# yuecideng/Misc3D

Hardware: AMD Instinct MI355X
Metric: RANSAC hypotheses/sec, 1M-pt cloud (inlier-score GB/s: roofline.algorithmic_reuse) (higher is better)
Workload: dtype f64 decisions (fp32 screen + fp64 recount)

## Files before the change

### include/misc3d_amd.h

```cpp
#ifndef MISC3D_AMD_H
#define MISC3D_AMD_H

#include <stddef.h>
#include <stdint.h>

#ifdef __cplusplus
extern "C" {
#endif

#define M3D_OK 1
#define M3D_FALSE 0
#define M3D_ERR_PROBABILITY (-1)
#define M3D_ERR_TOO_FEW_POINTS (-2)
#define M3D_ERR_NO_NORMALS (-3)
#define M3D_ERR_SIZE_MISMATCH (-4)
#define M3D_ERR_INVALID_ARG (-5)
#define M3D_ERR_DEVICE (-6)
#define M3D_ERR_INTERNAL (-7)

enum m3d_model_kind { M3D_PLANE = 0, M3D_SPHERE = 1, M3D_CYLINDER = 2 };

typedef struct m3d_stats {
    double fitness;
    double inlier_rmse;
// ... 326 lines not shown
    int32_t lead_hypotheses;
    int32_t score_groups_per_block;
    int32_t score_min_workgroups;
    int32_t dense_workgroups;
    int32_t reg_neighbour_lists;
    int32_t reg_prune;
    int32_t match_brute;
    int32_t match_fp32_screen;
    int32_t pool_limit_mb;
    int32_t kernel_timing;
    int32_t reg_sorted_lists;
    int32_t score_fp32_screen;
    int32_t cull_fp32;
    int32_t reg_fp32_screen;
    int32_t sorted_tombstones;
    int32_t score_mfma;
    int32_t score_mfma_groups;
    int32_t score_waves4;
    int32_t score_waves4_groups;
    int32_t score_phases;
    int32_t compact_one_pass;
    int32_t plane_bound;
    int32_t lanes;
    int32_t wait_spin_us;
    int32_t prestream;
    int32_t chunk_cap;
    int32_t first_chunk;
    int32_t reg_cells_per_radius;
    int32_t match_pipeline;
    int32_t reg_cache;
    int32_t device_aliases;
    int32_t lanes_eager;
    int32_t list_mask;
} m3d_config;
void m3d_get_config(m3d_config *out);
int m3d_set_config(const m3d_config *in);

const char *m3d_last_error(void);
int m3d_device_count(void);
const char *m3d_version(void);

#ifdef __cplusplus
}
#endif
#endif
```

### misc3d_amd/capi.py

```python
from __future__ import annotations

import ctypes as C
import threading
import os
import sys
from dataclasses import dataclass

import numpy as np

_HERE = os.path.dirname(os.path.abspath(__file__))
FP_ORDER = int(os.environ.get("M3D_FP_ORDER", "0") or 0)
_VARIANT = os.environ.get("M3D_LIB_VARIANT", "")
LIB_PATH = os.path.join(_HERE, "lib", *([_VARIANT] if _VARIANT else ([f"order{FP_ORDER}"] if FP_ORDER else [])), "libmisc3d_amd.so")
HEADER_PATH = os.path.join(os.path.dirname(_HERE), "include", "misc3d_amd.h")

PLANE, SPHERE, CYLINDER = 0, 1, 2
MINIMAL_SAMPLE = {PLANE: 3, SPHERE: 4, CYLINDER: 2}
NUM_PARAMS = {PLANE: 4, SPHERE: 4, CYLINDER: 7}
MODEL_STRIDE = 8

OK, FALSE = 1, 0
ERR_PROBABILITY, ERR_TOO_FEW_POINTS, ERR_NO_NORMALS, ERR_SIZE_MISMATCH = -1, -2, -3, -4
ERR_INVALID_ARG, ERR_DEVICE, ERR_INTERNAL = -5, -6, -7

# ... 173 lines not shown
                                                          C.c_void_p, C.c_int, C.c_size_t, C.c_void_p, C.c_void_p,
                                                          C.c_void_p, C.c_void_p, C.c_void_p]
        L.m3d_segment_plane_iterative_sharded.argtypes = [C.c_void_p, C.c_size_t, C.c_double, C.c_int, C.c_double,
                                                          C.c_void_p, C.c_int, C.c_void_p, C.c_size_t, C.c_void_p,
                                                          C.c_void_p, C.c_void_p, C.c_void_p]
        L.m3d_segment_plane_iterative_multi.argtypes = [C.c_void_p, C.c_size_t, C.c_double, C.c_int, C.c_double,
                                                        C.c_void_p, C.c_void_p, C.c_int, C.c_size_t, C.c_void_p,
                                                        C.c_void_p, C.c_void_p, C.c_void_p]
        L.m3d_fit_multi.argtypes = [C.c_int, C.c_void_p, C.c_void_p, C.c_size_t, C.c_double, C.c_size_t, C.c_double,
                                    C.c_void_p, C.c_void_p, C.c_int, C.c_void_p, C.c_void_p, C.c_void_p, C.c_void_p]
        L.m3d_registration_ransac_sharded.argtypes = [C.c_void_p, C.c_size_t, C.c_void_p, C.c_size_t, C.c_void_p,
                                                      C.c_void_p, C.c_size_t, C.c_double, C.c_int, C.c_double,
                                                      C.c_double, C.c_void_p, C.c_int, C.c_void_p, C.c_void_p,
                                                      C.c_void_p]
        L.m3d_bench_fp64_issue_rate.argtypes = [C.c_int, C.c_double, C.c_void_p, C.c_void_p]
        L.m3d_bench_cloud_setup_ms.argtypes = [C.c_void_p, C.c_void_p]
        L.m3d_bench_last_segment_ms.argtypes = [C.c_void_p]
        L.m3d_bench_reg_checkers.argtypes = [C.c_void_p, C.c_void_p, C.c_void_p, C.c_double, C.c_double]
        L.m3d_get_config.restype = None
        L.m3d_get_config.argtypes = [C.c_void_p]
        L.m3d_set_config.argtypes = [C.c_void_p]
        L.m3d_release_cached.restype = None
        L.m3d_release_cached.argtypes = [C.c_int]
        _lib = L
    return _lib


class Config(C.Structure):
    _fields_ = [(k, C.c_int32) for k in ("dense_scoring", "speculative_refine", "lead_hypotheses",
                                         "score_groups_per_block", "score_min_workgroups", "dense_workgroups",
                                         "reg_neighbour_lists", "reg_prune", "match_brute", "match_fp32_screen",
                                         "pool_limit_mb", "kernel_timing", "reg_sorted_lists", "score_fp32_screen",
                                         "cull_fp32", "reg_fp32_screen", "sorted_tombstones", "score_mfma", "score_mfma_groups", "score_waves4", "score_waves4_groups", "score_phases", "compact_one_pass", "plane_bound",
                                         "lanes", "wait_spin_us", "prestream", "chunk_cap", "first_chunk", "reg_cells_per_radius", "match_pipeline", "reg_cache", "device_aliases", "lanes_eager", "list_mask")]


def fp64_issue_rate(device=0, ms_target=2.0):
    t, ms = C.c_double(0), C.c_double(0)
    _check(lib().m3d_bench_fp64_issue_rate(device, ms_target, C.cast(C.byref(t), C.c_void_p), C.cast(C.byref(ms), C.c_void_p)))
    return float(t.value), float(ms.value)


def mfma_probe(xyz512, box, max_abs, records, device=0):
    xyz = np.ascontiguousarray(xyz512, dtype=np.float64).reshape(512, 3)
    bx = np.ascontiguousarray(box, dtype=np.float64).reshape(6)
    rec = np.zeros((len(records), 8), dtype=np.float64)
    rec[:, :5] = np.asarray(records, dtype=np.float64).reshape(-1, 5)
    q = np.empty((len(rec), 512, 2), dtype=np.float64)
    h = np.empty((len(rec), 3), dtype=np.float64)
    off = np.empty((512, 3), dtype=np.float32)
    f = lib().m3d_bench_mfma_probe
    f.restype = C.c_int
    f.argtypes = [C.c_int, C.c_void_p, C.c_void_p, C.c_double, C.c_void_p, C.c_size_t, C.c_void_p, C.c_void_p, C.c_void_p]
    _check(f(device, xyz.ctypes.data, bx.ctypes.data, float(max_abs), rec.ctypes.data, len(rec), q.ctypes.data, h.ctypes.data,
             off.ctypes.data))
    return q, h[:, 0].copy(), h[:, 1].copy(), h[:, 2].copy(), off


def match_last_path() -> int:
    f = lib().m3d_bench_match_last_path
    f.restype = C.c_uint
    f.argtypes = []
    return int(f())


def experimental() -> bool:
    f = lib().m3d_bench_experimental
# ... 1130 lines not shown
```

### misc3d_amd/csrc/m3d_config.cpp

```cpp
#include "m3d_config.hpp"

#include <algorithm>
#include <cstdlib>
#include <cstring>
#include <mutex>

#include "m3d_driver.hpp"

namespace m3d {
namespace {
m3d_config g_cfg;
std::once_flag g_once;
std::mutex g_cfg_mu;
thread_local m3d_config t_cfg;
thread_local int t_cfg_pins = 0;

long env_long(const char* name, long def) {
    const char* e = std::getenv(name);
    if (!e || !*e) return def;
    char* end = nullptr;
    const long v = std::strtol(e, &end, 10);
    return end == e ? def : v;
}
bool env_is(const char* name, char first) {
    const char* e = std::getenv(name);
    return e && e[0] == first;
}
void sanitize(m3d_config& c) {
    if (c.lead_hypotheses < 64 || c.lead_hypotheses % 64) c.lead_hypotheses = 128;
    if (c.score_groups_per_block < 1 || c.score_groups_per_block > 64) c.score_groups_per_block = 8;
    if (c.score_min_workgroups < 1) c.score_min_workgroups = 8192;
    if (c.dense_workgroups < 1) c.dense_workgroups = 8192;
    if (c.pool_limit_mb < 0) c.pool_limit_mb = 0;
    if (c.score_mfma_groups < 1 || c.score_mfma_groups > 64) c.score_mfma_groups = 64;
    if (c.score_waves4_groups < 1 || c.score_waves4_groups > 64) c.score_waves4_groups = 64;
    if (c.score_phases < -1 || c.score_phases == 1 || c.score_phases > 3) c.score_phases = -1;
    if (c.plane_bound < 0 || c.plane_bound > 2) c.plane_bound = 1;
    if (c.cull_fp32 < 0 || c.cull_fp32 > 2) c.cull_fp32 = 1;
    if (!kExperimentalBuild) c.score_mfma = c.score_waves4 = c.compact_one_pass = 0;
    if (c.lanes < 1 || c.lanes > 8) c.lanes = 4;
    if (c.wait_spin_us < 0) c.wait_spin_us = 500;
    c.prestream = c.prestream != 0;
    c.chunk_cap = (int32_t)std::min<long>(std::max<long>(((long)c.chunk_cap + 63) / 64 * 64, 1024), 262144);
    c.first_chunk = c.first_chunk <= 0 ? 0 : (int32_t)std::min<long>(((long)c.first_chunk + 63) / 64 * 64, 1 << 20);
    if (c.reg_cells_per_radius < 1 || c.reg_cells_per_radius > 16) c.reg_cells_per_radius = 4;
    if (c.match_pipeline < 0 || c.match_pipeline > 2) c.match_pipeline = 1;
    if (c.reg_cache < 0 || c.reg_cache > 2) c.reg_cache = 1;
    if (c.device_aliases < 0) c.device_aliases = 0;
    if (c.device_aliases > 16) c.device_aliases = 16;
    if (c.lanes_eager < 1 || c.lanes_eager > 8) c.lanes_eager = 2;
    if (c.list_mask < 0) c.list_mask = 1;
    if (c.list_mask > 16) c.list_mask = 16;
}
void load_env() {
    std::memset(&g_cfg, 0, sizeof(g_cfg));
    g_cfg.dense_scoring = env_is("M3D_DENSE", '1');
    g_cfg.speculative_refine = !env_is("M3D_SPEC", '0');
    g_cfg.lead_hypotheses = (int32_t)env_long("M3D_LEAD", 128);
    g_cfg.score_groups_per_block = (int32_t)env_long("M3D_GPB", 8);
    g_cfg.score_min_workgroups = (int32_t)env_long("M3D_SCORE_MIN_WGS", 8192);
    g_cfg.dense_workgroups = (int32_t)env_long("M3D_SCORE_WGS", 8192);
    g_cfg.reg_neighbour_lists = !env_is("M3D_REG_NL", '0');
    g_cfg.reg_prune = !env_is("M3D_REG_PRUNE", '0');
    g_cfg.match_brute = env_is("M3D_MATCH_BRUTE", '1');
    g_cfg.match_fp32_screen = env_is("M3D_MATCH_SCREEN", 'f');
    g_cfg.pool_limit_mb = (int32_t)env_long("M3D_POOL_MB", 4096);
    g_cfg.kernel_timing = env_is("M3D_KERNEL_TIMING", '1');
    g_cfg.reg_sorted_lists = !env_is("M3D_REG_SORTED", '0');
    g_cfg.score_fp32_screen = !env_is("M3D_SCORE_SCREEN", '0');
    g_cfg.cull_fp32 = env_is("M3D_CULL_FP32", '0') ? 0 : (env_is("M3D_CULL_FP32", '2') ? 2 : 1);
    g_cfg.reg_fp32_screen = !env_is("M3D_REG_SCREEN", '0');
    g_cfg.sorted_tombstones = !env_is("M3D_TOMBSTONES", '0');
    g_cfg.score_mfma = env_is("M3D_SCORE_MFMA", '1');
    g_cfg.score_mfma_groups = (int32_t)env_long("M3D_MFMA_GPB", 64);
    g_cfg.score_waves4 = env_is("M3D_SCORE_WAVES4", '1');
    g_cfg.score_waves4_groups = (int32_t)env_long("M3D_WAVES4_GPB", 64);
    g_cfg.score_phases = (int32_t)env_long("M3D_SCORE_PHASES", -1);
    g_cfg.compact_one_pass = env_is("M3D_COMPACT_ONE_PASS", '1');
    g_cfg.plane_bound = (int32_t)env_long("M3D_PLANE_BOUND", 1);
    g_cfg.lanes = (int32_t)env_long("M3D_LANES", 4);
    g_cfg.wait_spin_us = (int32_t)env_long("M3D_SPIN_US", 500);
    g_cfg.prestream = !env_is("M3D_PRESTREAM", '0');
    g_cfg.chunk_cap = (int32_t)env_long("M3D_CHUNK_CAP", 24576);
    g_cfg.first_chunk = (int32_t)env_long("M3D_FIRST_CHUNK", 2048);
    g_cfg.reg_cells_per_radius = (int32_t)env_long("M3D_REG_K", 4);
    g_cfg.match_pipeline = (int32_t)env_long("M3D_MATCH_PIPELINE", 1);
    g_cfg.reg_cache = (int32_t)env_long("M3D_REG_CACHE", 1);
    g_cfg.device_aliases = (int32_t)env_long("M3D_DEVICE_ALIASES", 0);
    g_cfg.lanes_eager = (int32_t)env_long("M3D_LANES_EAGER", 2);
    g_cfg.list_mask = (int32_t)env_long("M3D_LIST_MASK", 1);
    sanitize(g_cfg);
}
}

const m3d_config& config() {
    std::call_once(g_once, load_env);
    if (t_cfg_pins > 0) return t_cfg;
    std::lock_guard<std::mutex> lock(g_cfg_mu);
    t_cfg = g_cfg;
    return t_cfg;
}
void config_pin() {
    std::call_once(g_once, load_env);
    if (t_cfg_pins++ == 0) {
        std::lock_guard<std::mutex> lock(g_cfg_mu);
        t_cfg = g_cfg;
    }
}
void config_unpin() {
    if (t_cfg_pins > 0) --t_cfg_pins;
}
void config_store(const m3d_config& c) {
    std::call_once(g_once, load_env);
    m3d_config n = c;
    sanitize(n);
    std::lock_guard<std::mutex> lock(g_cfg_mu);
    g_cfg = n;
}
}

extern "C" {
void m3d_get_config(m3d_config* out) {
    if (out) *out = m3d::config();
// ... 12 lines not shown
```

### misc3d_amd/csrc/m3d_driver.hpp

```cpp
#pragma once
#include <hip/hip_runtime.h>

#include <cstddef>
#include <cstdint>
#include <functional>
#include <mutex>
#include <string>
#include <vector>

#include "../../include/misc3d_amd.h"
#include "m3d_cull_kernels.hpp"
#include "m3d_kernels.hpp"

struct m3d_cloud;

namespace m3d {

void set_error(const std::string& msg);
int fail(int code, const std::string& msg);

struct DevBuf {
    void* p = nullptr;
    size_t cap = 0;
    int dev = -1;
// ... 59 lines not shown
    uint32_t pick_seq = 0;
    const double* last_best_dev = nullptr;
    DevBuf cc_stage, cc_cell, cc_start, cc_fill, cc_sums, cc_total, cc_bbox;
    DevBuf pick;
    PinBuf h_pick;
    bool spec_compaction = false;
    uint64_t* idx_out_override = nullptr;
    bool defer_copy_sync = false;
    bool no_prune_hint = false;
    bool defer_refine = false;
    int refine_slot = 0;
    struct DeferredRefine {
        bool pending = false;
        int slot = 0;
        uint32_t ni = 0;
        double* params_out = nullptr;
    } deferred;
    PoisonJob pending_poison;
    bool poison_pending = false;
    uint64_t* poison_expected_at = nullptr, poison_pending_count = 0;
    DevBuf poison_total;
    bool ev_compact_early = false;
    bool spec_hit = false;
    PinBuf h_sums;
    DevBuf moment_partial;
    PinBuf h_moments;
    hipEvent_t ev_pre_gate = nullptr;
    uint32_t compact_epoch = 0;
    bool compaction_fused = false;
    uint64_t* compaction_idx_host = nullptr;
    bool compaction_mask = false;
    PinBuf h_mask, h_tile_counts;
    uint32_t mask_seq = 0;
    const std::function<const m3d::PartitionOut*(int64_t)>* partition_hook = nullptr;
    PinBuf h_best;
    PinBuf h_sync;
    PinBuf h_reg;
    uint32_t sync_seq = 0;
    DevBuf surv_list;
    hipEvent_t ev0 = nullptr, ev1 = nullptr;
    PinBuf h_match;
    std::vector<hipEvent_t> aux_events;
};

constexpr int kMaxLanes = 8;
struct MatchSide {
    const double* host;
    const double* dev;
    double max_abs;
};
int match_mutual_nn_on(DeviceCtx* ctx, const MatchSide& feat_src, size_t n_src, const MatchSide& feat_dst, size_t n_dst, int dim,
                       size_t* out_src, size_t* out_dst, size_t* k_out);
int device_max_abs(DeviceCtx* ctx, const double* dev, size_t n, double* out);
int registration_ransac_on(DeviceCtx* ctx, m3d_cloud* csrc, m3d_cloud* cdst, const double* src, size_t n_src,
                           const double* dst, size_t n_dst, const size_t* corr_src, const size_t* corr_dst, size_t m,
                           double threshold, int max_iter, double edge_length_threshold, double confidence,
                           const uint64_t* seed, double* T_out, m3d_reg_stats* stats,
                           m3d_reg** session_out = nullptr );
int information_matrix_on(DeviceCtx* ctx, m3d_cloud* csrc, m3d_cloud* cdst, const double* dst, size_t n_dst,
                          double max_correspondence_distance, const double* T, double* info, uint64_t* n_correspondences,
                          m3d_reg* session = nullptr);
void reg_session_release(m3d_reg* q);

void dev_pool_trim(int device);
int logical_device_count();
int physical_device(int logical);
// ... 82 lines not shown
```

### misc3d_amd/csrc/m3d_kernels.hip

```cpp
#include <cstdio>
#include <cstdlib>
#include "m3d_kernels.hpp"
#include "m3d_config.hpp"
#include "m3d_poison.hpp"

#include "m3d_fp.hpp"

#pragma clang fp contract(off)

namespace m3d {

__global__ __launch_bounds__(256) void aos_to_soa_k(const double* __restrict__ aos,
                                                     double* __restrict__ x, double* __restrict__ y,
                                                     double* __restrict__ z, uint32_t n,
                                                     uint32_t n_pad) {
    const uint32_t i = blockIdx.x * 256u + threadIdx.x;
    if (i >= n_pad) return;
    const double nan = u2f(0x7FF8000000000000ull);
    double px = nan, py = nan, pz = nan;
    if (i < n) {
        px = aos[3 * (size_t)i];
        py = aos[3 * (size_t)i + 1];
        pz = aos[3 * (size_t)i + 2];
    }
// ... 324 lines not shown
}

void launch_reduce_partials(const uint32_t* partial, uint32_t n_tiles, uint32_t h_pad,
                            uint32_t* counts, hipStream_t s) {
    if (h_pad == 0 || n_tiles == 0) return;
    const dim3 g(h_pad / 64, (n_tiles + kReduceTilesPerBlock - 1) / kReduceTilesPerBlock), b(256);
    reduce_partials_k<<<g, b, 0, s>>>(partial, n_tiles, h_pad, counts);
}

template <int NV>
__device__ __forceinline__ void block_tree_reduce(double (&acc)[NV], double* sm ) {
    for (int k = 0; k < NV; ++k) sm[k * 256 + threadIdx.x] = acc[k];
    __syncthreads();
    for (int off = 128; off > 0; off >>= 1) {
        if ((int)threadIdx.x < off)
            for (int k = 0; k < NV; ++k) sm[k * 256 + threadIdx.x] += sm[k * 256 + threadIdx.x + off];
        __syncthreads();
    }
}

template <int KIND>
__device__ __forceinline__ double ref_distance(const double* m, double x, double y, double z) {
    if (KIND == 0) return plane_distance(m, x, y, z);
    if (KIND == 1) return sphere_distance(m, x, y, z);
    return cylinder_distance(m, x, y, z);
}

template <int KIND, bool SUMS>
__global__ __launch_bounds__(256) void compact_count_k(CloudView c, const double* __restrict__ model,
                                                        double thr, int invert,
                                                        uint32_t* __restrict__ block_counts,
                                                        double* __restrict__ model_copy,
                                                        double* __restrict__ moment_partial,
                                                        uint64_t* __restrict__ mask_host = nullptr) {
    __shared__ uint32_t wsum[4];
    __shared__ unsigned long long wmask[kCompactTile / 64];
    double m[kModelStride];
    for (int k = 0; k < kModelStride; ++k) m[k] = model[k];
    if (model_copy && blockIdx.x == 0 && threadIdx.x < kModelStride) model_copy[threadIdx.x] = model[threadIdx.x];
    const int lane = threadIdx.x & 63, wave = threadIdx.x >> 6;
    uint32_t cnt = 0;
    const uint32_t base = blockIdx.x * kCompactTile;
    constexpr int NV = KIND == 1 ? 12 : 9;
    double acc[NV];
    for (int k = 0; k < NV; ++k) acc[k] = 0.0;
    const double c0x = KIND == 0 ? m[4] : m[0], c0y = KIND == 0 ? m[5] : m[1], c0z = KIND == 0 ? m[6] : m[2];
    for (int r = 0; r < kCompactTile / 256; ++r) {
        const uint32_t i = base + r * 256 + threadIdx.x;
        bool f = false;
        if (i < c.n) {
            const double px = c.x[i], py = c.y[i], pz = c.z[i];
            const double d = ref_distance<KIND>(m, px, py, pz);
            f = (d < thr) != (invert != 0) && (invert != 2 || px == px);
            if (SUMS && f) {
                const double sx = px - c0x, sy = py - c0y, sz = pz - c0z;
                acc[0] += sx;
                acc[1] += sy;
                acc[2] += sz;
                acc[3] += sx * sx;
                acc[4] += sx * sy;
                acc[5] += sx * sz;
                acc[6] += sy * sy;
                acc[7] += sy * sz;
                acc[8] += sz * sz;
                if (KIND == 1) {
                    const double q = (sx * sx + sy * sy) + sz * sz;
                    acc[9] += sx * q;
                    acc[10] += sy * q;
                    acc[11] += sz * q;
                }
            }
        }
        const unsigned long long b = __ballot(f);
        cnt += (uint32_t)__popcll(b);
        if (lane == 0) wmask[r * 4 + wave] = b;
    }
    if (lane == 0) wsum[wave] = cnt;
    __syncthreads();
    if (threadIdx.x == 0) block_counts[blockIdx.x] = (wsum[0] + wsum[1]) + (wsum[2] + wsum[3]);
    if (mask_host && threadIdx.x < kCompactTile / 64)
        mask_host[(size_t)blockIdx.x * (kCompactTile / 64) + threadIdx.x] = wmask[threadIdx.x];
    if (SUMS) {
        __shared__ double sm[NV * 256];
        __syncthreads();
        block_tree_reduce<NV>(acc, sm);
        if (threadIdx.x < 12) moment_partial[(size_t)blockIdx.x * 16 + threadIdx.x] = (int)threadIdx.x < NV ? sm[threadIdx.x * 256] : 0.0;
    }
}

__global__ __launch_bounds__(1024) void scan_blocks_k(uint32_t* __restrict__ v, uint32_t nb,
                                                       uint32_t* __restrict__ total,
                                                       const double* __restrict__ moment_partial,
                                                       double* __restrict__ moment_out,
                                                       uint32_t* __restrict__ total_host ) {
    __shared__ uint32_t buf[1024];
    __shared__ uint32_t carry;
    __shared__ double msum[12 * 64];
    if (moment_partial) {
        const uint32_t g = threadIdx.x >> 6, l = threadIdx.x & 63;
        if (g < 12) {
            double a = 0.0;
            for (uint32_t b = l; b < nb; b += 64) a += moment_partial[(size_t)b * 16 + g];
            msum[g * 64 + l] = a;
        }
        __syncthreads();
        for (int off = 32; off > 0; off >>= 1) {
            if (g < 12 && (int)l < off) msum[g * 64 + l] += msum[g * 64 + l + off];
            __syncthreads();
        }
        if (threadIdx.x < 12) moment_out[threadIdx.x] = msum[threadIdx.x * 64];
    }
    if (threadIdx.x == 0) carry = 0;
// ... 196 lines not shown
                oy[pos] = py[r];
                oz[pos] = pz[r];
                if (MODE == 2) oorig[pos] = og[r];
            }
        }
        if (MODE == 4 && ((bg[r] >> lane) & 1ull)) {
            const uint32_t pos = rest_base + woff2 + (uint32_t)__popcll(bg[r] & below);
            ox[pos] = px[r];
            oy[pos] = py[r];
            oz[pos] = pz[r];
            oorig[pos] = og[r];
        }
        row_base += (wf[r][0] + wf[r][1]) + (wf[r][2] + wf[r][3]);
        if (MODE == 4) rest_base += (wg[r][0] + wg[r][1]) + (wg[r][2] + wg[r][3]);
    }
    if (tile == gridDim.x - 1 && threadIdx.x == 0) compact_tail_total(tail, row_base);
    if ((MODE == 2 || MODE == 3 || MODE == 4) && tile == gridDim.x - 1) {
        const uint32_t n = MODE == 4 ? rest_base : row_base;
        const uint32_t n_pad = min(n_pad_cap, (n + kScoreTile - 1) / kScoreTile * kScoreTile);
        const double nan = u2f(0x7FF8000000000000ull);
        for (uint32_t i = n + threadIdx.x; i < n_pad; i += 256u) {
            ox[i] = nan;
            oy[i] = nan;
            oz[i] = nan;
        }
    }
    if (SUMS && tile == gridDim.x - 1) {
        __threadfence();
        fold_moment_partials(tail);
    }
}

__global__ __launch_bounds__(256) void compact_mask_tail_k(const uint32_t* __restrict__ block_counts, CompactTail tail,
                                                            uint32_t* __restrict__ counts_host, uint32_t* done_word,
                                                            uint32_t done_seq) {
    __shared__ uint32_t wsum[4];
    const int lane = threadIdx.x & 63, wave = threadIdx.x >> 6;
    uint32_t part = 0;
    for (uint32_t i = threadIdx.x; i < tail.nb; i += 256u) {
        const uint32_t v = block_counts[i];
        counts_host[i] = v;
        part += v;
    }
    for (int off = 32; off > 0; off >>= 1) part += (uint32_t)__shfl_xor((int)part, off, 64);
    if (lane == 0) wsum[wave] = part;
    if (tail.moment_partial) fold_moment_partials(tail);
    else __syncthreads();
    if (threadIdx.x == 0) compact_tail_total(tail, (wsum[0] + wsum[1]) + (wsum[2] + wsum[3]));
    if (done_word) {
        __threadfence_system();
        __syncthreads();
        if (threadIdx.x == 0) __hip_atomic_store(done_word, done_seq, __ATOMIC_RELEASE, __HIP_MEMORY_SCOPE_SYSTEM);
    }
}

template <int KIND>
static void launch_compact_kind(const CloudView& c, const double* model, double thr, int mode,
                                const uint32_t* orig, uint64_t* out_idx, double* out_dist,
                                double* ox, double* oy, double* oz, uint32_t* oorig,
                                uint32_t n_pad_out, const CompactScratch& scratch, uint32_t* total,
                                hipStream_t s, double* model_copy, double* moment_partial, double* moment_out,
                                uint64_t* out_idx_host, uint32_t* total_host, const PartitionOut* part,
                                uint64_t* mask_host, uint32_t* counts_host, uint32_t* done_word, uint32_t done_seq) {
    const uint32_t nb = (c.n + kCompactTile - 1) / kCompactTile;
    if (nb == 0) {
        (void)hipMemsetAsync(total, 0, sizeof(uint32_t), s);
        if (total_host) (void)hipMemcpyAsync(total_host, total, sizeof(uint32_t), hipMemcpyDeviceToHost, s);
        if (model_copy) (void)hipMemcpyAsync(model_copy, model, sizeof(double) * kModelStride, hipMemcpyDeviceToHost, s);
        if (moment_out) (void)hipMemsetAsync(moment_out, 0, sizeof(double) * 13, s);
        return;
    }
    const bool sums = moment_partial && moment_out && mode == 0 && KIND != 2;
    const bool one = kExperimentalBuild && config().compact_one_pass != 0 && nb <= kCompactOnePassMaxTiles && scratch.tag != 0u;
    uint32_t* block_counts = scratch.slots;
    const uint32_t tag = scratch.tag;
    if (mask_host && counts_host && sums && !orig && !part && !one) {
        compact_count_k<KIND == 2 ? 0 : KIND, true><<<nb, 256, 0, s>>>(c, model, thr, 0, block_counts, model_copy, moment_partial,
                                                                       mask_host);
        CompactTail tail;
        tail.total = total;
        tail.total_host = total_host;
        tail.moment_partial = moment_partial;
        tail.moment_out = moment_out;
        tail.nb = nb;
        compact_mask_tail_k<<<1, 256, 0, s>>>(block_counts, tail, counts_host, done_word, done_seq);
        return;
    }
    if (!one) {
        if (sums)
            compact_count_k<KIND == 2 ? 0 : KIND, true><<<nb, 256, 0, s>>>(c, model, thr, 0, block_counts, model_copy, moment_partial);
        else
            compact_count_k<KIND, false><<<nb, 256, 0, s>>>(c, model, thr, mode == 3 ? 2 : (mode >= 2 ? 1 : 0), block_counts, model_copy, nullptr);
    }
    CompactTail tail;
    tail.total = total;
    tail.total_host = total_host;
    tail.moment_partial = sums ? moment_partial : nullptr;
    tail.moment_out = sums ? moment_out : nullptr;
    tail.nb = nb;
    const PartitionOut none;
    const PartitionOut& po = part ? *part : none;
    constexpr int KS = KIND == 2 ? 0 : KIND;
#define M3D_COMPACT_GO(MODE_, ONE_, SUMS_, K_, ...) \
    compact_write_k<K_, MODE_, ONE_, SUMS_><<<nb, 256, 0, s>>>(c, model, thr, __VA_ARGS__, tail, model_copy, moment_partial)
#define M3D_COMPACT_PICK(MODE_, WITH_SUMS_, ...)                                              \
    do {                                                                                      \
        if constexpr (kExperimentalBuild) {                                                   \
            if constexpr (WITH_SUMS_) {                                                       \
                if (one && sums) {                                                            \
                    M3D_COMPACT_GO(MODE_, true, true, KS, __VA_ARGS__);                       \
                    break;                                                                    \
                }                                                                             \
            }                                                                                 \
            if (one) {                                                                        \
                M3D_COMPACT_GO(MODE_, true, false, KIND, __VA_ARGS__);                        \
                break;                                                                        \
            }                                                                                 \
        }                                                                                     \
        M3D_COMPACT_GO(MODE_, false, false, KIND, __VA_ARGS__);                               \
    } while (0)
    if (mode == 0 && part && orig)
        M3D_COMPACT_PICK(4, true, orig, block_counts, tag, out_idx, nullptr, po.ox, po.oy, po.oz, po.oorig, po.n_pad_cap, out_idx_host);
    else if (mode == 0)
        M3D_COMPACT_PICK(0, true, orig, block_counts, tag, out_idx, nullptr, nullptr, nullptr, nullptr, nullptr, 0u, out_idx_host);
    else if (mode == 1)
        M3D_COMPACT_PICK(1, false, orig, block_counts, tag, nullptr, out_dist, nullptr, nullptr, nullptr, nullptr, 0u, nullptr);
    else if (mode == 2)
        M3D_COMPACT_PICK(2, false, orig, block_counts, tag, nullptr, nullptr, ox, oy, oz, oorig, n_pad_out, nullptr);
    else
        M3D_COMPACT_PICK(3, false, nullptr, block_counts, tag, nullptr, nullptr, ox, oy, oz, nullptr, n_pad_out, nullptr);
#undef M3D_COMPACT_PICK
#undef M3D_COMPACT_GO
}

void launch_compact(int kind, const CloudView& c, const double* model, double thr, int mode,
                    const uint32_t* orig, uint64_t* out_idx, double* out_dist, double* ox,
                    double* oy, double* oz, uint32_t* oorig, uint32_t n_pad_out,
                    const CompactScratch& scratch, uint32_t* total, hipStream_t s, double* model_copy,
                    double* moment_partial, double* moment_out, uint64_t* out_idx_host, uint32_t* total_host,
                    const PartitionOut* part, uint64_t* mask_host, uint32_t* counts_host, uint32_t* done_word,
                    uint32_t done_seq) {
    if (kind == 0)
        launch_compact_kind<0>(c, model, thr, mode, orig, out_idx, out_dist, ox, oy, oz, oorig, n_pad_out, scratch, total, s,
                               model_copy, moment_partial, moment_out, out_idx_host, total_host, part, mask_host, counts_host, done_word, done_seq);
    else if (kind == 1)
        launch_compact_kind<1>(c, model, thr, mode, orig, out_idx, out_dist, ox, oy, oz, oorig, n_pad_out, scratch, total, s,
                               model_copy, moment_partial, moment_out, out_idx_host, total_host, part, mask_host, counts_host, done_word, done_seq);
    else
        launch_compact_kind<2>(c, model, thr, mode, orig, out_idx, out_dist, ox, oy, oz, oorig, n_pad_out, scratch, total, s,
                               model_copy, nullptr, nullptr, out_idx_host, total_host, part, nullptr, nullptr, nullptr, 0u);
}

__global__ void gather_points_k(CloudView c, const uint64_t* __restrict__ idx, size_t total, double* __restrict__ out) {
    const size_t i = (size_t)blockIdx.x * 256u + threadIdx.x;
    if (i >= total) return;
    const uint64_t j = idx[i];
    out[3 * i] = c.x[j];
    out[3 * i + 1] = c.y[j];
    out[3 * i + 2] = c.z[j];
}
void launch_gather_points(const CloudView& c, const uint64_t* idx, size_t total, double* out, hipStream_t s) {
    if (total) gather_points_k<<<(uint32_t)((total + 255) / 256), 256, 0, s>>>(c, idx, total, out);
}

__global__ __launch_bounds__(64) void serial_sum_k(const double* __restrict__ v,
                                                    const uint32_t* __restrict__ n_ptr,
                                                    double* __restrict__ out) {
    __shared__ double buf[2][1024];
    const uint32_t n = n_ptr[0];
    const uint32_t lane = threadIdx.x;
    double s = 0.0;
    double r[16];
#pragma unroll
    for (int j = 0; j < 16; ++j) {
        const uint32_t i = (uint32_t)j * 64u + lane;
        r[j] = i < n ? v[i] : 0.0;
    }
    int cur = 0;
    for (uint32_t b0 = 0; b0 < n; b0 += 1024u) {
#pragma unroll
        for (int j = 0; j < 16; ++j) buf[cur][j * 64 + lane] = r[j];
        __builtin_amdgcn_fence(__ATOMIC_RELEASE, "workgroup");
        __builtin_amdgcn_wave_barrier();
// ... 206 lines not shown
```

### misc3d_amd/csrc/m3d_kernels.hpp

```cpp
#pragma once
#include <hip/hip_runtime.h>

#include <cstddef>
#include <cstdint>

namespace m3d {

constexpr int kModelStride = 8;
constexpr int kScoreP = 8;
constexpr int kScoreBlock = 256;
constexpr int kScoreTile = kScoreBlock * kScoreP;
constexpr int kCompactTile = 2048;

#ifdef M3D_EXPERIMENTAL
constexpr bool kExperimentalBuild = true;
#else
constexpr bool kExperimentalBuild = false;
#endif

struct CloudView {
    const double* x;
    const double* y;
    const double* z;
    const double* nx;
// ... 40 lines not shown
                  uint32_t h_splits, uint32_t* partial, hipStream_t s);
void launch_reduce_partials(const uint32_t* partial, uint32_t n_tiles, uint32_t h_pad,
                            uint32_t* counts, hipStream_t s);

constexpr int kBboxPartialDoubles = 1024 * 8;
void launch_bbox(const double* x, const double* y, const double* z, uint32_t n, double* partial, double* out,
                 hipStream_t s);

constexpr uint32_t kCompactOnePassMaxTiles = 1024;
constexpr uint32_t kCompactEpochs = 0xFFFFFu;
struct CompactScratch {
    uint32_t* slots = nullptr;
    uint32_t tag = 0;
};
struct PartitionOut {
    double *ox = nullptr, *oy = nullptr, *oz = nullptr;
    uint32_t* oorig = nullptr;
    uint32_t n_pad_cap = 0;
};
void launch_gather_points(const CloudView& c, const uint64_t* idx, size_t total, double* out, hipStream_t s);
void launch_compact(int kind, const CloudView& c, const double* model, double thr, int mode,
                    const uint32_t* orig, uint64_t* out_idx, double* out_dist, double* ox,
                    double* oy, double* oz, uint32_t* oorig, uint32_t n_pad_out,
                    const CompactScratch& scratch, uint32_t* total, hipStream_t s,
                    double* model_copy = nullptr ,
                    double* moment_partial = nullptr ,
                    double* moment_out = nullptr ,
                    uint64_t* out_idx_host = nullptr ,
                    uint32_t* total_host = nullptr ,
                    const PartitionOut* part = nullptr ,
                    uint64_t* mask_host = nullptr ,
                    uint32_t* counts_host = nullptr ,
                    uint32_t* done_word = nullptr ,
                    uint32_t done_seq = 0);
constexpr int kFusedMomentDoubles = 16;
void moments_about_mean(const double* moment_out, const double c0[3], double n, double mean[3], double centred[10]);

void launch_serial_sum(const double* v, const uint32_t* n, double* out, hipStream_t s);

constexpr int kSumPartialDoubles = 256 * 16;
constexpr int kGeneralFitHostDoubles = 256 * 16 + 4;
void launch_general_fit_sums(const CloudView& c, const uint64_t* idx, uint32_t n_idx, double* partial_dev,
                             double* out_host, hipStream_t s);
void general_fit_sums_finish(const double* out_host, double* sums14);

constexpr int kErrorSumScratchDoubles = 1024 * 4;
void launch_error_sum(int kind, const CloudView& c, const double* model_a, const double* model_b, double thr,
                      double* partial, uint32_t* ticket, double* out_host, hipStream_t s);

void launch_scan_blocks(uint32_t* v, uint32_t nb, uint32_t* total, hipStream_t s);

void launch_fp64_issue_probe(double* out, int blocks, int iters, hipStream_t s);

void launch_iota(uint32_t* v, uint32_t n, hipStream_t s);

}
```

### misc3d_amd/csrc/m3d_mt19937.hpp

```cpp
#pragma once
#include <cstdint>

#if defined(__HIP_DEVICE_COMPILE__)
#define M3D_HOST_SIMD_CLONES
#else
#define M3D_HOST_SIMD_CLONES __attribute__((target_clones("default", "avx2", "avx512f")))
#endif

namespace m3d {

struct Mt19937Mod {
    static constexpr int kN = 624;
    uint32_t mt[kN];
    uint32_t out[kN];
    int pos = kN;
    uint32_t d = 0, magic = 0, shift = 0;

    void seed(uint32_t s) {
        mt[0] = s;
        for (uint32_t i = 1; i < (uint32_t)kN; ++i) mt[i] = 1812433253u * (mt[i - 1] ^ (mt[i - 1] >> 30)) + i;
        pos = kN;
    }
    void set_modulus(uint32_t divisor) {
        d = divisor;
        uint32_t L = 0;
        while ((UINT64_C(1) << L) < d) ++L;
        magic = (uint32_t)(((UINT64_C(1) << 32) * ((UINT64_C(1) << L) - d)) / d + 1);
        shift = L ? L - 1 : 0;
    }
    M3D_HOST_SIMD_CLONES void refill() {
        auto tw = [](uint32_t a, uint32_t b, uint32_t c) {
            const uint32_t y = (a & 0x80000000u) | (b & 0x7fffffffu);
            return c ^ (y >> 1) ^ ((0u - (y & 1u)) & 0x9908b0dfu);
        };
        for (int i = 0; i < 227; ++i) mt[i] = tw(mt[i], mt[i + 1], mt[i + 397]);
        for (int i = 227; i < 623; ++i) mt[i] = tw(mt[i], mt[i + 1], mt[i - 227]);
        mt[623] = tw(mt[623], mt[0], mt[396]);
        const uint32_t dd = d, mg = magic, sh = shift;
        for (int i = 0; i < kN; ++i) {
            uint32_t y = mt[i];
            y ^= y >> 11;
            y ^= (y << 7) & 0x9d2c5680u;
            y ^= (y << 15) & 0xefc60000u;
            y ^= y >> 18;
            const uint32_t t = (uint32_t)(((uint64_t)mg * y) >> 32);
            const uint32_t q = (((y - t) >> 1) + t) >> sh;
            out[i] = dd == 1u ? 0u : y - q * dd;
        }
        pos = 0;
    }
    uint32_t next() {
        if (pos == kN) refill();
        return out[pos++];
    }
    template <int M>
    void fill(uint32_t* s, size_t n_hyp) {
        for (size_t h = 0; h < n_hyp; ++h, s += M) {
            if (pos + M <= kN) {
                const uint32_t* p = out + pos;
                bool distinct = true;
                for (int k = 1; k < M; ++k)
                    for (int j = 0; j < k; ++j) distinct = distinct && (p[k] != p[j]);
                if (distinct) {
                    for (int k = 0; k < M; ++k) s[k] = p[k];
                    pos += M;
                    continue;
                }
            }
            int valid = 0;
            while (valid < M) {
                const uint32_t idx = next();
                bool dup = false;
                for (int k = 0; k < valid; ++k) dup = dup || (s[k] == idx);
                if (!dup) s[valid++] = idx;
            }
        }
    }
};

}
```

### misc3d_amd/csrc/m3d_refine.cpp

```cpp
#include "m3d_driver_internal.hpp"
#include "m3d_mask_expand.hpp"

#include <condition_variable>
#include <mutex>
#include <sched.h>

#pragma clang fp contract(off)

namespace m3d {

namespace {
class MaskPool {
public:
    static MaskPool& get() {
        static MaskPool* p = new MaskPool();
        return *p;
    }
    static uint32_t writer_cap() {
        const int lm = config().list_mask;
        uint32_t cap = lm >= 2 ? (uint32_t)lm : 8u;
        cpu_set_t set;
        CPU_ZERO(&set);
        if (sched_getaffinity(0, sizeof(set), &set) == 0) cap = std::min<uint32_t>(cap, (uint32_t)std::max(CPU_COUNT(&set), 1));
        return std::max<uint32_t>(cap, 1u);
// ... 221 lines not shown
        double acc = A[r][3];
        for (int k = r + 1; k < 3; ++k) acc -= A[r][k] * c[k];
        c[r] = A[r][r] != 0.0 ? acc / A[r][r] : 0.0;
    }
    const double w3 = s[9] / n;
    out[0] = mean[0] + c[0];
    out[1] = mean[1] + c[1];
    out[2] = mean[2] + c[2];
    out[3] = std::sqrt(((c[0] * c[0] + c[1] * c[1]) + c[2] * c[2]) + w3);
    return true;
}


static uint64_t* idx_dev(DeviceCtx* ctx) { return ctx->idx_out_override ? ctx->idx_out_override : ctx->idx.as<uint64_t>(); }
int refine_slot(const DeviceCtx* ctx) { return ctx->defer_refine ? ctx->refine_slot : 0; }
double* h_best_at(DeviceCtx* ctx) { return ctx->h_best.as<double>() + (size_t)refine_slot(ctx) * kModelStride; }
uint8_t* h_total_at(DeviceCtx* ctx) { return ctx->h_pick.as<uint8_t>() + 64 + 8 * refine_slot(ctx); }
static double* h_moments_at(DeviceCtx* ctx) { return ctx->h_moments.as<double>() + (size_t)refine_slot(ctx) * kFusedMomentDoubles; }

int issue_refine_compaction(DeviceCtx* ctx, const CloudView& flag_view, const uint32_t* orig_dev, int kind,
                                   double thr, const double* model_dev, const double* lazy_in, void* total_host,
                                   bool fused, uint64_t* idx_host, const PartitionOut* part, bool allow_mask) {
    const uint32_t n = flag_view.n;
    const uint32_t nb = (n + kCompactTile - 1) / kCompactTile;
    RESERVE(ctx->idx, sizeof(uint64_t) * (size_t)std::max<uint32_t>(n, 1));
    CompactScratch scratch;
    if (const int rc = compact_scratch(ctx, nb, &scratch); rc != M3D_OK) return rc;
    RESERVE(ctx->total, sizeof(uint32_t) * 4);
    fused = fused && kind != M3D_CYLINDER;
    if (fused) {
        RESERVE(ctx->moment_partial, sizeof(double) * 16 * (size_t)std::max<uint32_t>(nb, 1));
        RESERVE(ctx->h_moments, sizeof(double) * 2 * kFusedMomentDoubles);
    }
    const bool mask = allow_mask && fused && idx_host && nb && !orig_dev && !part && !ctx->idx_out_override &&
                      !ctx->defer_refine && config().list_mask != 0;
    if (mask) {
        RESERVE(ctx->h_mask, sizeof(uint64_t) * kMaskTileWords * (size_t)nb);
        RESERVE(ctx->h_tile_counts, sizeof(uint32_t) * (size_t)nb);
        if (!ctx->h_sync.p) {
            RESERVE(ctx->h_sync, 64);
            std::memset(ctx->h_sync.p, 0, 64);
        }
        if (++ctx->mask_seq == 0) ++ctx->mask_seq;
        MaskPool::get().arm();
    }
    launch_compact(kind, flag_view, model_dev, thr, 0, orig_dev,
                   idx_dev(ctx), nullptr,
                   nullptr, nullptr, nullptr, nullptr, 0, scratch,
                   ctx->total.as<uint32_t>(), ctx->stream, const_cast<double*>(lazy_in),
                   fused ? ctx->moment_partial.as<double>() : nullptr, fused ? h_moments_at(ctx) : nullptr,
                   idx_host, static_cast<uint32_t*>(total_host) , part,
                   mask ? ctx->h_mask.as<uint64_t>() : nullptr, mask ? ctx->h_tile_counts.as<uint32_t>() : nullptr,
                   mask ? ctx->h_sync.as<uint32_t>() + 1 : nullptr, ctx->mask_seq);
    ctx->compaction_fused = fused;
    ctx->compaction_idx_host = idx_host;
    ctx->compaction_mask = mask;
    return M3D_OK;
}

static bool expand_compaction_mask(DeviceCtx* ctx, uint32_t n, uint32_t expected, uint64_t* dst) {
    const uint32_t nb = (n + kCompactTile - 1) / kCompactTile;
    const uint32_t* counts = ctx->h_tile_counts.as<const uint32_t>();
    uint64_t total = 0;
    for (uint32_t t = 0; t < nb; ++t) total += counts[t];
    if (total != expected) return false;
    return MaskPool::get().expand(ctx->h_mask.as<const uint64_t>(), n, counts, dst);
}

int refine(DeviceCtx* ctx, const CloudView& flag_view, const CloudView& gather_view,
                  const uint32_t* orig_dev, int kind, double thr, const double* model_dev,
                  double* params_host , size_t* inliers,
                  size_t* n_inliers, int* general_fit_ok, int64_t expected_ni,
                  const std::function<int(int64_t)>* before_wait,
                  const double* lazy_in ,
                  const void* compaction_total ,
                  bool fused ) {
    const uint32_t n = flag_view.n;
    fused = fused && lazy_in != nullptr;
    RESERVE(ctx->sums, sizeof(double) * 32);
    RESERVE(ctx->sum_partial, sizeof(double) * kSumPartialDoubles);
    RESERVE(ctx->h_sums, sizeof(double) * kGeneralFitHostDoubles);
    RESERVE(ctx->h_small, 256);
    uint8_t* h = ctx->h_small.as<uint8_t>();
    const uint8_t* h_total = compaction_total ? static_cast<const uint8_t*>(compaction_total) : h;
    if (!compaction_total) {
        uint64_t* idx_host = inliers && fused && !ctx->idx_out_override &&
                                     is_library_pinned(inliers, sizeof(uint64_t) * (size_t)std::max<uint32_t>(n, 1))
                                 ? reinterpret_cast<uint64_t*>(inliers) : nullptr;
        const PartitionOut* part = ctx->partition_hook && orig_dev ? (*ctx->partition_hook)(expected_ni) : nullptr;
// ... 4 lines not shown
    const bool have_moments = fused && ctx->compaction_fused;
    const bool idx_on_host = inliers && ctx->compaction_idx_host == reinterpret_cast<uint64_t*>(inliers);
    if (ctx->compaction_mask && !(idx_on_host && expected_ni >= 0 && (uint64_t)expected_ni <= n))
        return refine(ctx, flag_view, gather_view, orig_dev, kind, thr, model_dev, params_host, inliers, n_inliers,
                      general_fit_ok, -1, before_wait, lazy_in, nullptr, false);
    if (expected_ni >= 0 && (uint64_t)expected_ni <= n) {
        const uint32_t ni_e = (uint32_t)expected_ni;
        const bool need_fit_e = kind != M3D_CYLINDER && ni_e >= (kind == M3D_PLANE ? 3u : 4u);
        if (!(compaction_total && ctx->ev_compact_early)) HIPCHK(hipEventRecord(ctx->ev_compact, ctx->stream));
        ctx->ev_compact_early = false;
        const bool early_copy = !idx_on_host && inliers && ni_e && is_library_pinned(inliers, sizeof(uint64_t) * (size_t)ni_e);
        if (early_copy) {
            HIPCHK(hipStreamWaitEvent(copy_stream_of(ctx), ctx->ev_compact, 0));
            HIPCHK(hipMemcpyAsync(inliers, (void*)idx_dev(ctx),
                                  sizeof(uint64_t) * (size_t)ni_e, hipMemcpyDeviceToHost, copy_stream_of(ctx)));
        }
        if (need_fit_e && !have_moments) {
            launch_general_fit_sums(gather_view, idx_dev(ctx), ni_e, ctx->sum_partial.as<double>(),
                                    ctx->h_sums.as<double>(), ctx->stream);
        }
        bool hooked = false;
        if (before_wait) {
            const int hr = (*before_wait)(expected_ni);
            before_wait = nullptr;
            hooked = true;
            if (hr != M3D_OK) return hr;
        }
        if (inliers && ni_e && !early_copy && !idx_on_host) {
            HIPCHK(hipStreamWaitEvent(copy_stream_of(ctx), ctx->ev_compact, 0));
            HIPCHK(hipMemcpyAsync(inliers, (void*)idx_dev(ctx),
                                  sizeof(uint64_t) * (size_t)ni_e, hipMemcpyDeviceToHost, copy_stream_of(ctx)));
        }
        HIPCHK(hipGetLastError());
        if (hooked && (have_moments || !need_fit_e)) {
            HIPCHK(hipEventSynchronize(ctx->ev_compact));
        } else if (ctx->compaction_mask && !hooked) {
            const int wrc = word_wait_spin(ctx, ctx->h_sync.as<uint32_t>() + 1, ctx->mask_seq);
            if (wrc != M3D_OK) return wrc;
        } else {
            const int wrc = stream_wait_spin(ctx);
            if (wrc != M3D_OK) return wrc;
        }
        const bool list_on_copy_stream = inliers && ni_e && !idx_on_host;
        if (list_on_copy_stream && !(ctx->defer_copy_sync && ctx->idx_out_override)) HIPCHK(hipStreamSynchronize(copy_stream_of(ctx)));
        if (lazy_in) std::memcpy(params_host, lazy_in, sizeof(double) * kModelStride);
        uint32_t ni_chk;
        std::memcpy(&ni_chk, h_total, 4);
        if (ni_chk != ni_e ||
            (ctx->compaction_mask && ni_e && !expand_compaction_mask(ctx, n, ni_e, reinterpret_cast<uint64_t*>(inliers))))
            return refine(ctx, flag_view, gather_view, orig_dev, kind, thr, model_dev, params_host, inliers, n_inliers,
                          general_fit_ok, -1, nullptr, nullptr, nullptr);
        *n_inliers = ni_e;
        *general_fit_ok = 1;
        if (kind != M3D_CYLINDER) {
            if (!need_fit_e) {
                *general_fit_ok = 0;
            } else {
                double sums[14];
                double mean[3];
                if (have_moments) {
                    const double* rec = lazy_in;
                    const double c0[3] = {kind == M3D_PLANE ? rec[4] : rec[0], kind == M3D_PLANE ? rec[5] : rec[1],
                                          kind == M3D_PLANE ? rec[6] : rec[2]};
                    moments_about_mean(h_moments_at(ctx), c0, (double)ni_e, mean, sums + 4);
                } else {
                    general_fit_sums_finish(ctx->h_sums.as<double>(), sums);
                    for (int k = 0; k < 3; ++k) mean[k] = sums[k] / (double)ni_e;
                }
                double out[4];
                const bool ok = kind == M3D_PLANE ? plane_from_moments(mean, sums + 4, out)
                                                  : sphere_from_moments(mean, sums + 4, (double)ni_e, out);
                if (ok)
                    std::memcpy(params_host, out, sizeof(out));
                else
                    *general_fit_ok = 0;
            }
        }
        return M3D_OK;
    }
    HIPCHK(hipGetLastError());
    if (before_wait) {
        const int hr = (*before_wait)(-1);
// ... 92 lines not shown
```

Before: 45.72 million.

## Expand inlier mask on host while tail kernel runs; batch MT19937 sample fills

The count kernel now writes per-tile counts straight to pinned host memory. The tail kernel sets a ready flag as its first action, so the host can expand the compaction mask into the inlier list while the tail reduction and moment finish are still running. Separately, the MT19937 hypothesis fill checks a whole run of generated indices for repeats with a branch-free masked scan and bulk-copies it, instead of testing each hypothesis individually. This risks extra host spin-waits and a redundant expansion if the count check later fails.

```diff
diff --git a/include/misc3d_amd.h b/include/misc3d_amd.h
--- a/include/misc3d_amd.h
+++ b/include/misc3d_amd.h
@@ -382,6 +382,7 @@
     int32_t device_aliases;
     int32_t lanes_eager;
     int32_t list_mask;
+    int32_t mask_early;
 } m3d_config;
 void m3d_get_config(m3d_config *out);
 int m3d_set_config(const m3d_config *in);
diff --git a/misc3d_amd/capi.py b/misc3d_amd/capi.py
--- a/misc3d_amd/capi.py
+++ b/misc3d_amd/capi.py
@@ -229,7 +229,7 @@
                                          "reg_neighbour_lists", "reg_prune", "match_brute", "match_fp32_screen",
                                          "pool_limit_mb", "kernel_timing", "reg_sorted_lists", "score_fp32_screen",
                                          "cull_fp32", "reg_fp32_screen", "sorted_tombstones", "score_mfma", "score_mfma_groups", "score_waves4", "score_waves4_groups", "score_phases", "compact_one_pass", "plane_bound",
-                                         "lanes", "wait_spin_us", "prestream", "chunk_cap", "first_chunk", "reg_cells_per_radius", "match_pipeline", "reg_cache", "device_aliases", "lanes_eager", "list_mask")]
+                                         "lanes", "wait_spin_us", "prestream", "chunk_cap", "first_chunk", "reg_cells_per_radius", "match_pipeline", "reg_cache", "device_aliases", "lanes_eager", "list_mask", "mask_early")]
 
 
 def fp64_issue_rate(device=0, ms_target=2.0):
diff --git a/misc3d_amd/csrc/m3d_config.cpp b/misc3d_amd/csrc/m3d_config.cpp
--- a/misc3d_amd/csrc/m3d_config.cpp
+++ b/misc3d_amd/csrc/m3d_config.cpp
@@ -51,6 +51,7 @@
     if (c.lanes_eager < 1 || c.lanes_eager > 8) c.lanes_eager = 2;
     if (c.list_mask < 0) c.list_mask = 1;
     if (c.list_mask > 16) c.list_mask = 16;
+    c.mask_early = c.mask_early != 0;
 }
 void load_env() {
     std::memset(&g_cfg, 0, sizeof(g_cfg));
@@ -89,6 +90,7 @@
     g_cfg.device_aliases = (int32_t)env_long("M3D_DEVICE_ALIASES", 0);
     g_cfg.lanes_eager = (int32_t)env_long("M3D_LANES_EAGER", 2);
     g_cfg.list_mask = (int32_t)env_long("M3D_LIST_MASK", 1);
+    g_cfg.mask_early = !env_is("M3D_MASK_EARLY", '0');
     sanitize(g_cfg);
 }
 }
diff --git a/misc3d_amd/csrc/m3d_driver.hpp b/misc3d_amd/csrc/m3d_driver.hpp
--- a/misc3d_amd/csrc/m3d_driver.hpp
+++ b/misc3d_amd/csrc/m3d_driver.hpp
@@ -115,6 +115,7 @@
     bool compaction_mask = false;
     PinBuf h_mask, h_tile_counts;
     uint32_t mask_seq = 0;
+    bool compaction_mask_early = false;
     const std::function<const m3d::PartitionOut*(int64_t)>* partition_hook = nullptr;
     PinBuf h_best;
     PinBuf h_sync;
diff --git a/misc3d_amd/csrc/m3d_kernels.hip b/misc3d_amd/csrc/m3d_kernels.hip
--- a/misc3d_amd/csrc/m3d_kernels.hip
+++ b/misc3d_amd/csrc/m3d_kernels.hip
@@ -380,7 +380,8 @@
                                                         uint32_t* __restrict__ block_counts,
                                                         double* __restrict__ model_copy,
                                                         double* __restrict__ moment_partial,
-                                                        uint64_t* __restrict__ mask_host = nullptr) {
+                                                        uint64_t* __restrict__ mask_host = nullptr,
+                                                        uint32_t* __restrict__ counts_host = nullptr) {
     __shared__ uint32_t wsum[4];
     __shared__ unsigned long long wmask[kCompactTile / 64];
     double m[kModelStride];
@@ -425,7 +426,11 @@
     }
     if (lane == 0) wsum[wave] = cnt;
     __syncthreads();
-    if (threadIdx.x == 0) block_counts[blockIdx.x] = (wsum[0] + wsum[1]) + (wsum[2] + wsum[3]);
+    if (threadIdx.x == 0) {
+        const uint32_t mine = (wsum[0] + wsum[1]) + (wsum[2] + wsum[3]);
+        block_counts[blockIdx.x] = mine;
+        if (counts_host) counts_host[blockIdx.x] = mine;
+    }
     if (mask_host && threadIdx.x < kCompactTile / 64)
         mask_host[(size_t)blockIdx.x * (kCompactTile / 64) + threadIdx.x] = wmask[threadIdx.x];
     if (SUMS) {
@@ -688,14 +693,15 @@
 }
 
 __global__ __launch_bounds__(256) void compact_mask_tail_k(const uint32_t* __restrict__ block_counts, CompactTail tail,
-                                                            uint32_t* __restrict__ counts_host, uint32_t* done_word,
-                                                            uint32_t done_seq) {
+                                                            uint32_t* __restrict__ counts_host, uint32_t* ready_word,
+                                                            uint32_t* done_word, uint32_t done_seq) {
     __shared__ uint32_t wsum[4];
+    if (ready_word && threadIdx.x == 0) __hip_atomic_store(ready_word, done_seq, __ATOMIC_RELEASE, __HIP_MEMORY_SCOPE_SYSTEM);
     const int lane = threadIdx.x & 63, wave = threadIdx.x >> 6;
     uint32_t part = 0;
     for (uint32_t i = threadIdx.x; i < tail.nb; i += 256u) {
         const uint32_t v = block_counts[i];
-        counts_host[i] = v;
+        if (counts_host) counts_host[i] = v;
         part += v;
     }
     for (int off = 32; off > 0; off >>= 1) part += (uint32_t)__shfl_xor((int)part, off, 64);
@@ -717,7 +723,8 @@
                                 uint32_t n_pad_out, const CompactScratch& scratch, uint32_t* total,
                                 hipStream_t s, double* model_copy, double* moment_partial, double* moment_out,
                                 uint64_t* out_idx_host, uint32_t* total_host, const PartitionOut* part,
-                                uint64_t* mask_host, uint32_t* counts_host, uint32_t* done_word, uint32_t done_seq) {
+                                uint64_t* mask_host, uint32_t* counts_host, uint32_t* done_word, uint32_t done_seq,
+                                uint32_t* ready_word) {
     const uint32_t nb = (c.n + kCompactTile - 1) / kCompactTile;
     if (nb == 0) {
         (void)hipMemsetAsync(total, 0, sizeof(uint32_t), s);
@@ -732,14 +739,14 @@
     const uint32_t tag = scratch.tag;
     if (mask_host && counts_host && sums && !orig && !part && !one) {
         compact_count_k<KIND == 2 ? 0 : KIND, true><<<nb, 256, 0, s>>>(c, model, thr, 0, block_counts, model_copy, moment_partial,
-                                                                       mask_host);
+                                                                       mask_host, ready_word ? counts_host : nullptr);
         CompactTail tail;
         tail.total = total;
         tail.total_host = total_host;
         tail.moment_partial = moment_partial;
         tail.moment_out = moment_out;
         tail.nb = nb;
-        compact_mask_tail_k<<<1, 256, 0, s>>>(block_counts, tail, counts_host, done_word, done_seq);
+        compact_mask_tail_k<<<1, 256, 0, s>>>(block_counts, tail, ready_word ? nullptr : counts_host, ready_word, done_word, done_seq);
         return;
     }
     if (!one) {
@@ -795,16 +802,16 @@
                     const CompactScratch& scratch, uint32_t* total, hipStream_t s, double* model_copy,
                     double* moment_partial, double* moment_out, uint64_t* out_idx_host, uint32_t* total_host,
                     const PartitionOut* part, uint64_t* mask_host, uint32_t* counts_host, uint32_t* done_word,
-                    uint32_t done_seq) {
+                    uint32_t done_seq, uint32_t* ready_word) {
     if (kind == 0)
         launch_compact_kind<0>(c, model, thr, mode, orig, out_idx, out_dist, ox, oy, oz, oorig, n_pad_out, scratch, total, s,
-                               model_copy, moment_partial, moment_out, out_idx_host, total_host, part, mask_host, counts_host, done_word, done_seq);
+                               model_copy, moment_partial, moment_out, out_idx_host, total_host, part, mask_host, counts_host, done_word, done_seq, ready_word);
     else if (kind == 1)
         launch_compact_kind<1>(c, model, thr, mode, orig, out_idx, out_dist, ox, oy, oz, oorig, n_pad_out, scratch, total, s,
-                               model_copy, moment_partial, moment_out, out_idx_host, total_host, part, mask_host, counts_host, done_word, done_seq);
+                               model_copy, moment_partial, moment_out, out_idx_host, total_host, part, mask_host, counts_host, done_word, done_seq, ready_word);
     else
         launch_compact_kind<2>(c, model, thr, mode, orig, out_idx, out_dist, ox, oy, oz, oorig, n_pad_out, scratch, total, s,
-                               model_copy, nullptr, nullptr, out_idx_host, total_host, part, nullptr, nullptr, nullptr, 0u);
+                               model_copy, nullptr, nullptr, out_idx_host, total_host, part, nullptr, nullptr, nullptr, 0u, nullptr);
 }
 
 __global__ void gather_points_k(CloudView c, const uint64_t* __restrict__ idx, size_t total, double* __restrict__ out) {
diff --git a/misc3d_amd/csrc/m3d_kernels.hpp b/misc3d_amd/csrc/m3d_kernels.hpp
--- a/misc3d_amd/csrc/m3d_kernels.hpp
+++ b/misc3d_amd/csrc/m3d_kernels.hpp
@@ -96,7 +96,8 @@
                     uint64_t* mask_host = nullptr ,
                     uint32_t* counts_host = nullptr ,
                     uint32_t* done_word = nullptr ,
-                    uint32_t done_seq = 0);
+                    uint32_t done_seq = 0,
+                    uint32_t* ready_word = nullptr );
 constexpr int kFusedMomentDoubles = 16;
 void moments_about_mean(const double* moment_out, const double c0[3], double n, double mean[3], double centred[10]);
 
diff --git a/misc3d_amd/csrc/m3d_mt19937.hpp b/misc3d_amd/csrc/m3d_mt19937.hpp
--- a/misc3d_amd/csrc/m3d_mt19937.hpp
+++ b/misc3d_amd/csrc/m3d_mt19937.hpp
@@ -1,5 +1,8 @@
 #pragma once
+#include <algorithm>
+#include <cstddef>
 #include <cstdint>
+#include <cstring>
 
 #if defined(__HIP_DEVICE_COMPILE__)
 #define M3D_HOST_SIMD_CLONES
@@ -9,10 +12,23 @@
 
 namespace m3d {
 
+struct Mt19937RepeatMasks {
+    uint32_t mask[3][3][624];
+    Mt19937RepeatMasks() {
+        for (int m = 2; m <= 4; ++m)
+            for (int j = 1; j <= 3; ++j)
+                for (int i = 0; i < 624; ++i) mask[m - 2][j - 1][i] = (i % m) + j < m ? ~0u : 0u;
+    }
+};
+inline const Mt19937RepeatMasks& mt19937_repeat_masks() {
+    static const Mt19937RepeatMasks t;
+    return t;
+}
+
 struct Mt19937Mod {
     static constexpr int kN = 624;
     uint32_t mt[kN];
-    uint32_t out[kN];
+    uint32_t out[kN + 4] = {};
     int pos = kN;
     uint32_t d = 0, magic = 0, shift = 0;
 
@@ -53,27 +69,64 @@
         if (pos == kN) refill();
         return out[pos++];
     }
+    M3D_HOST_SIMD_CLONES static bool run_has_repeat(const uint32_t* p, int len, int m, const Mt19937RepeatMasks& t) {
+        const uint32_t *m1 = t.mask[m - 2][0], *m2 = t.mask[m - 2][1], *m3 = t.mask[m - 2][2];
+        uint32_t acc = 0;
+        if (m == 2) {
+            for (int i = 0; i < len; ++i) acc |= (0u - (uint32_t)(p[i] == p[i + 1])) & m1[i];
+        } else if (m == 3) {
+            for (int i = 0; i < len; ++i)
+                acc |= ((0u - (uint32_t)(p[i] == p[i + 1])) & m1[i]) | ((0u - (uint32_t)(p[i] == p[i + 2])) & m2[i]);
+        } else {
+            for (int i = 0; i < len; ++i)
+                acc |= ((0u - (uint32_t)(p[i] == p[i + 1])) & m1[i]) | ((0u - (uint32_t)(p[i] == p[i + 2])) & m2[i]) |
+                       ((0u - (uint32_t)(p[i] == p[i + 3])) & m3[i]);
+        }
+        return acc != 0;
+    }
     template <int M>
     void fill(uint32_t* s, size_t n_hyp) {
-        for (size_t h = 0; h < n_hyp; ++h, s += M) {
-            if (pos + M <= kN) {
-                const uint32_t* p = out + pos;
-                bool distinct = true;
-                for (int k = 1; k < M; ++k)
-                    for (int j = 0; j < k; ++j) distinct = distinct && (p[k] != p[j]);
-                if (distinct) {
-                    for (int k = 0; k < M; ++k) s[k] = p[k];
-                    pos += M;
-                    continue;
-                }
+        static_assert(M >= 2 && M <= 4, "run_has_repeat's masks");
+        const Mt19937RepeatMasks& masks = mt19937_repeat_masks();
+        size_t h = 0;
+        while (h < n_hyp) {
+            const size_t run = std::min<size_t>((size_t)(kN - pos) / M, n_hyp - h);
+            if (run && !run_has_repeat(out + pos, (int)(run * M), M, masks)) {
+                std::memcpy(s, out + pos, sizeof(uint32_t) * run * M);
+                pos += (int)(run * M);
+                s += run * M;
+                h += run;
+                continue;
             }
-            int valid = 0;
-            while (valid < M) {
-                const uint32_t idx = next();
-                bool dup = false;
-                for (int k = 0; k < valid; ++k) dup = dup || (s[k] == idx);
-                if (!dup) s[valid++] = idx;
+            for (const size_t stop = h + std::max<size_t>(run, 1); h < stop;) {
+                const int before = pos;
+                fill_one<M>(s);
+                ++h;
+                s += M;
+                if (pos < before) break;
             }
+        }
+    }
+
+    template <int M>
+    void fill_one(uint32_t* s) {
+        if (pos + M <= kN) {
+            const uint32_t* p = out + pos;
+            bool distinct = true;
+            for (int k = 1; k < M; ++k)
+                for (int j = 0; j < k; ++j) distinct = distinct && (p[k] != p[j]);
+            if (distinct) {
+                for (int k = 0; k < M; ++k) s[k] = p[k];
+                pos += M;
+                return;
+            }
+        }
+        int valid = 0;
+        while (valid < M) {
+            const uint32_t idx = next();
+            bool dup = false;
+            for (int k = 0; k < valid; ++k) dup = dup || (s[k] == idx);
+            if (!dup) s[valid++] = idx;
         }
     }
 };
diff --git a/misc3d_amd/csrc/m3d_refine.cpp b/misc3d_amd/csrc/m3d_refine.cpp
--- a/misc3d_amd/csrc/m3d_refine.cpp
+++ b/misc3d_amd/csrc/m3d_refine.cpp
@@ -277,6 +277,7 @@
         RESERVE(ctx->moment_partial, sizeof(double) * 16 * (size_t)std::max<uint32_t>(nb, 1));
         RESERVE(ctx->h_moments, sizeof(double) * 2 * kFusedMomentDoubles);
     }
+    const bool early = config().mask_early != 0;
     const bool mask = allow_mask && fused && idx_host && nb && !orig_dev && !part && !ctx->idx_out_override &&
                       !ctx->defer_refine && config().list_mask != 0;
     if (mask) {
@@ -296,10 +297,12 @@
                    fused ? ctx->moment_partial.as<double>() : nullptr, fused ? h_moments_at(ctx) : nullptr,
                    idx_host, static_cast<uint32_t*>(total_host) , part,
                    mask ? ctx->h_mask.as<uint64_t>() : nullptr, mask ? ctx->h_tile_counts.as<uint32_t>() : nullptr,
-                   mask ? ctx->h_sync.as<uint32_t>() + 1 : nullptr, ctx->mask_seq);
+                   mask ? ctx->h_sync.as<uint32_t>() + 1 : nullptr, ctx->mask_seq,
+                   mask && early ? ctx->h_sync.as<uint32_t>() + 2 : nullptr);
     ctx->compaction_fused = fused;
     ctx->compaction_idx_host = idx_host;
     ctx->compaction_mask = mask;
+    ctx->compaction_mask_early = mask && early;
     return M3D_OK;
 }
 
@@ -370,9 +373,16 @@
                                   sizeof(uint64_t) * (size_t)ni_e, hipMemcpyDeviceToHost, copy_stream_of(ctx)));
         }
         HIPCHK(hipGetLastError());
+        bool expanded = false, expand_ok = true;
         if (hooked && (have_moments || !need_fit_e)) {
             HIPCHK(hipEventSynchronize(ctx->ev_compact));
         } else if (ctx->compaction_mask && !hooked) {
+            if (ctx->compaction_mask_early && ni_e) {
+                const int erc = word_wait_spin(ctx, ctx->h_sync.as<uint32_t>() + 2, ctx->mask_seq);
+                if (erc != M3D_OK) return erc;
+                expand_ok = expand_compaction_mask(ctx, n, ni_e, reinterpret_cast<uint64_t*>(inliers));
+                expanded = true;
+            }
             const int wrc = word_wait_spin(ctx, ctx->h_sync.as<uint32_t>() + 1, ctx->mask_seq);
             if (wrc != M3D_OK) return wrc;
         } else {
@@ -385,7 +395,8 @@
         uint32_t ni_chk;
         std::memcpy(&ni_chk, h_total, 4);
         if (ni_chk != ni_e ||
-            (ctx->compaction_mask && ni_e && !expand_compaction_mask(ctx, n, ni_e, reinterpret_cast<uint64_t*>(inliers))))
+            (ctx->compaction_mask && ni_e &&
+             !(expanded ? expand_ok : expand_compaction_mask(ctx, n, ni_e, reinterpret_cast<uint64_t*>(inliers)))))
             return refine(ctx, flag_view, gather_view, orig_dev, kind, thr, model_dev, params_host, inliers, n_inliers,
                           general_fit_ok, -1, nullptr, nullptr, nullptr);
         *n_inliers = ni_e;
```

Result: faster. 50.24 million, median of 6 (+9.9%).
